# DJjjjhao/FIRA-ICSE

Measured on AMD Instinct MI355X. Metric: training commits/sec (FIRA default config), higher is better.
Workload: dtype f32; 1 GPU; BASELINE configs[1]: FIRA training step (fwd+bwd+Adam, dropout 0.1/0.2), batch 32 commits/GPU, fp32, 650-node graphs (mean nnz 1066/graph), vocab 24650; global_batch=32, parallelism=dp1

## Files before the change

### fira_icse_amd/csrc/attention.hip

```cpp
#include "engine.h"
#include "epilogue.h"
#include "mfma_frag.h"

namespace fira {

constexpr float SQRT_DH = 5.656854249492381f;
constexpr float INV_SQRT_DH = 1.0f / SQRT_DH;
constexpr int MAX_TK = 384;

constexpr float LOG2E = 1.4426950408889634f;
constexpr float SCORE2 = INV_SQRT_DH * LOG2E;
constexpr float MASKED2 = -1e9f * LOG2E;
__device__ __forceinline__ constexpr int acc_c(int s) { return (s & 3) + 8 * (s >> 2); }
__device__ __forceinline__ uint32_t low_bits(int n) { return n <= 0 ? 0u : (n >= 32 ? 0xffffffffu : (1u << n) - 1u); }
__device__ __forceinline__ float bit_select(int sel, float a, float b) {
    return __int_as_float((sel & __float_as_int(a)) | (~sel & __float_as_int(b)));
}
__device__ __forceinline__ int bit_of(uint32_t word, int c) { return __builtin_amdgcn_sbfe((int)word, c, 1); }

__device__ __forceinline__ void buf_frag(float (&f)[16], rsrc_t r, unsigned off) {
#pragma unroll
    for (int i = 0; i < 4; ++i) {
        const f32x4v v = __builtin_bit_cast(f32x4v, __builtin_amdgcn_raw_buffer_load_b128(r, off + 16u * i, 0, 0));
        f[4 * i + 0] = v.x; f[4 * i + 1] = v.y; f[4 * i + 2] = v.z; f[4 * i + 3] = v.w;
    }
}
__device__ __forceinline__ void buf_rows(float (&f)[16], rsrc_t r, unsigned off0, unsigned ld4) {
#pragma unroll
    for (int s = 0; s < 16; ++s) f[s] = buf_load_f32(r, off0 + (unsigned)acc_c(s) * ld4);
}
__device__ __forceinline__ rsrc_t rows_rsrc(const float* base, int n, int ld) {
    return buf_rsrc(base, n > 0 ? (unsigned)(n - 1) * (unsigned)ld * 4u + 128u : 0u);
}

struct AttnRanges { int qb, tq, k0, tk; };
// ... 646 lines not shown
                       ldv, key_valid, causal, q_pos0, O, ldo, kb, kvb, qpk, q_off, self_kv, k_off)
    if (Tk <= 32) { if (bf16) FIRA_ATT_FWD(1, true); else FIRA_ATT_FWD(1, false); }
    else { if (bf16) FIRA_ATT_FWD(12, true); else FIRA_ATT_FWD(12, false); }
#undef FIRA_ATT_FWD
    FIRA_CHECK_LAUNCH("attention_fwd");
    return 0;
}
int attention_fwd(hipStream_t s, int B, int H, int Tq, int Tk, const float* Q, int ldq, const float* K, int ldk,
                  const float* V, int ldv, const int32_t* key_valid, int causal, int q_pos0, float* O, int ldo,
                  const int32_t* q_off, int self_kv, int bf16, const int32_t* k_off) {
    return attention_fwd_ex(s, B, H, Tq, Tk, Q, ldq, K, ldk, V, ldv, key_valid, causal, q_pos0, O, ldo, Tk, Tk, 1, q_off, self_kv,
                            bf16, k_off);
}

int attention_bwd(hipStream_t s, int B, int H, int Tq, int Tk, const float* Q, int ldq, const float* K, int ldk,
                  const float* V, int ldv, const int32_t* key_valid, int causal, int q_pos0, const float* O, int ldo,
                  const float* dO, int lddo, float* dQ, int lddq, float* dK, int lddk, float* dV, int lddv,
                  const int32_t* q_off, int self_kv, int bf16, const int32_t* k_off) {
    ProfScope prof(s, PROF_ATTN, 0.0);
    if (B <= 0) return 0;
    if (int e = check_geometry("attention_bwd", Tq, Tk, ldq, ldk, ldv, Q, K, V)) return e;
    FIRA_REQUIRE(ldo % 4 == 0 && lddo % 4 == 0 && (uintptr_t)O % 16 == 0 && (uintptr_t)dO % 16 == 0,
                 "attention_bwd: O/dO rows must be 16-byte aligned");
#define FIRA_ATT_BWD(NW_, BF_)                                                                                      \
    hipLaunchKernelGGL((attention_bwd_kernel<NW_, BF_>), dim3(B * H), dim3(NW_ * 64), 0, s, H, Tq, Tk, Q, ldq, K, ldk, V, \
                       ldv, key_valid, causal, q_pos0, O, ldo, dO, lddo, dQ, lddq, dK, lddk, dV, lddv, q_off, self_kv, k_off)
    if (Tk <= 32) { if (bf16) FIRA_ATT_BWD(1, true); else FIRA_ATT_BWD(1, false); }
    else { if (bf16) FIRA_ATT_BWD(12, true); else FIRA_ATT_BWD(12, false); }
#undef FIRA_ATT_BWD
    FIRA_CHECK_LAUNCH("attention_bwd");
    return 0;
}

}

extern "C" {
int fira_attention_fwd(void* stream, int B, int H, int Tq, int Tk, const float* Q, int ldq, const float* K, int ldk,
                       const float* V, int ldv, const int32_t* key_valid, int causal, int q_pos0, float* O, int ldo) {
    return fira::attention_fwd((hipStream_t)stream, B, H, Tq, Tk, Q, ldq, K, ldk, V, ldv, key_valid, causal, q_pos0, O,
                               ldo);
}
int fira_decode_attention(void* stream, int BR, int H, int Tk, const float* Q, int ldq, const float* K, int ldk,
                          const float* V, int ldv, const int32_t* key_valid, float* O, int ldo, int kb, int kvb, int qpk,
                          const float* Knew, const float* Vnew, int ldn, float* Kc_out, float* Vc_out,
                          const int32_t* k_off) {
    FIRA_REQUIRE(Q && K && V && key_valid && O, "fira_decode_attention: null pointer argument");
    return fira::decode_attention((hipStream_t)stream, BR, H, Tk, Q, ldq, K, ldk, V, ldv, key_valid, O, ldo, kb, kvb, qpk, Knew,
                                  Vnew, ldn, Kc_out, Vc_out, k_off);
}
int fira_attention_bwd(void* stream, int B, int H, int Tq, int Tk, const float* Q, int ldq, const float* K, int ldk,
                       const float* V, int ldv, const int32_t* key_valid, int causal, int q_pos0, const float* O,
                       int ldo, const float* dO, int lddo, float* dQ, int lddq, float* dK, int lddk, float* dV,
                       int lddv) {
    return fira::attention_bwd((hipStream_t)stream, B, H, Tq, Tk, Q, ldq, K, ldk, V, ldv, key_valid, causal, q_pos0, O,
                               ldo, dO, lddo, dQ, lddq, dK, lddk, dV, lddv);
}
int fira_attention_fwd_ex(void* stream, int B, int H, int Tq, int Tk, const float* Q, int ldq, const float* K, int ldk,
                          const float* V, int ldv, const int32_t* key_valid, int causal, int q_pos0, float* O, int ldo,
                          const int32_t* q_off, int self_kv, int dtype, const int32_t* k_off) {
    FIRA_REQUIRE(dtype == FIRA_F32 || dtype == FIRA_BF16, "fira_attention_fwd_ex: dtype must be FIRA_F32 or FIRA_BF16");
    FIRA_REQUIRE(!(k_off && self_kv), "fira_attention_fwd_ex: k_off (ragged memory rows) and self_kv exclude each other");
    return fira::attention_fwd((hipStream_t)stream, B, H, Tq, Tk, Q, ldq, K, ldk, V, ldv, key_valid, causal, q_pos0, O,
                               ldo, q_off, self_kv, dtype == FIRA_BF16, k_off);
}
int fira_attention_bwd_ex(void* stream, int B, int H, int Tq, int Tk, const float* Q, int ldq, const float* K, int ldk,
                          const float* V, int ldv, const int32_t* key_valid, int causal, int q_pos0, const float* O,
// ... 9 lines not shown
```

### fira_icse_amd/csrc/engine.h

```cpp
#pragma once
#include "common.h"
#include <string>
#include <vector>

namespace fira {

int gemm_f32(hipStream_t s, int tA, int tB, int M, int N, int K, const float* A, int lda, const float* B, int ldb,
             float* C, int ldc, const float* bias, int flags, int splitk);
int gemm_f32_ex(hipStream_t s, int tA, int tB, int M, int N, int K, const float* A, int lda, const float* B, int ldb,
                float* C, int ldc, const float* bias, int flags, int splitk, float* colsum,
                const int32_t* c_rows = nullptr, const float* relu_mask = nullptr);
int gemm_bf16_ex(hipStream_t s, int tA, int tB, int M, int N, int K, const float* A, int lda, const float* B, int ldb,
                 float* C, int ldc, const float* bias, int flags, int splitk, float* colsum,
                 const int32_t* c_rows = nullptr, const float* relu_mask = nullptr);
struct ShadowEntry { int64_t offset; int rows, cols, pitch_t; int64_t offset_t; };
constexpr int SHADOW_MAX = 64;
struct ShadowTable {
    int n = 0;
    int64_t wbt_elems = 0;
    int tile_start[SHADOW_MAX + 1] = {0};
    ShadowEntry e[SHADOW_MAX];
};
int weight_shadows(hipStream_t s, const ShadowTable& tab, const float* P, uint16_t* Wb, uint16_t* WbT);
int gemm_bf16_wb_ex(hipStream_t s, int M, int N, int K, const float* A, int lda, const uint16_t* Bb, int ldb, float* C,
// ... 133 lines not shown
int node_features(hipStream_t s, int Nc, const int32_t* node_rows, int N, int L, int S, const int32_t* sou,
                  const int32_t* sub, const int32_t* ast, const float* emb, const float* ast_emb, const float* pos_code,
                  float* X, const int32_t* slot2 = nullptr, float* X2 = nullptr,
                  const AdamRowsView* vw = nullptr);
int rows_move(hipStream_t s, int mode, int R, int W, float* out, const float* in, const int32_t* src, const int32_t* dst);
int rows_move_ld(hipStream_t s, int mode, int R, int W, float* out, int ld_out, const float* in, int ld_in,
                 const int32_t* src, const int32_t* dst);
int rows_gather_idx(hipStream_t s, int R, float* compact, const float* src, const int32_t* rows);
int rows_scatter_add_idx(hipStream_t s, int R, const float* compact, float* dst, const int32_t* rows);
int fill_pos_tables(hipStream_t s, int L, float* pos_code, int T, float* pos_tar);
int tar_mask(hipStream_t s, int n, const int32_t* tar, int32_t* valid);
int permute_cache(hipStream_t s, int nl, int BR, int T, int len, const int32_t* parent, const float* ksrc,
                  const float* vsrc, float* kdst, float* vdst, const int32_t* hist_src, int32_t* hist_dst);
int mark_history(hipStream_t s, int BR, int T, int step, const int32_t* tokens, int32_t* hist);
int decode_embed(hipStream_t s, int BR, int T, int step, const int32_t* tokens, const float* table, const float* pos_row,
                 float* x, int32_t* hist);

int attention_fwd(hipStream_t s, int B, int H, int Tq, int Tk, const float* Q, int ldq, const float* K, int ldk,
                  const float* V, int ldv, const int32_t* key_valid, int causal, int q_pos0, float* O, int ldo,
                  const int32_t* q_off = nullptr, int self_kv = 0,
                  int bf16 = 0,
                  const int32_t* k_off = nullptr);
int attention_fwd_ex(hipStream_t s, int B, int H, int Tq, int Tk, const float* Q, int ldq, const float* K, int ldk,
                     const float* V, int ldv, const int32_t* key_valid, int causal, int q_pos0, float* O, int ldo,
                     int kb, int kvb, int qpk, const int32_t* q_off = nullptr, int self_kv = 0, int bf16 = 0,
                     const int32_t* k_off = nullptr);
int decode_attention(hipStream_t s, int BR, int H, int Tk, const float* Q, int ldq, const float* K, int ldk,
                     const float* V, int ldv, const int32_t* key_valid, float* O, int ldo, int kb, int kvb, int qpk,
                     const float* Knew = nullptr, const float* Vnew = nullptr, int ldn = 0, float* Kc_out = nullptr,
                     float* Vc_out = nullptr, const int32_t* k_off = nullptr);
int decode_self_block(hipStream_t s, int BR, int Tk, int T, const float* qkv, float* Kc, float* Vc, const int32_t* hist,
                      const float* WoT, const float* bo, const float* xres, const float* gamma, const float* beta,
                      const float* WqT, const float* bq, float* xa, float* qc);
int decode_attention_kv16(hipStream_t s, int BR, int H, int Tk, const float* Q, int ldq, const uint16_t* K, int ldk,
                          const uint16_t* V, int ldv, const int32_t* key_valid, float* O, int ldo, int kb, int kvb, int qpk,
                          const int32_t* k_off = nullptr);
int rows_to_bf16(hipStream_t s, int64_t n, const float* in, uint16_t* out);
int rows_from_bf16(hipStream_t s, int64_t n, const uint16_t* in, float* out);
int attention_bwd(hipStream_t s, int B, int H, int Tq, int Tk, const float* Q, int ldq, const float* K, int ldk,
                  const float* V, int ldv, const int32_t* key_valid, int causal, int q_pos0, const float* O, int ldo,
                  const float* dO, int lddo, float* dQ, int lddq, float* dK, int lddk, float* dV, int lddv,
                  const int32_t* q_off = nullptr, int self_kv = 0, int bf16 = 0, const int32_t* k_off = nullptr);
int copy_score_fwd(hipStream_t s, int B, int T, int S, const float* src, const float* tgt, const float* w,
                   const float* bias, float* score);
int copy_score_fwd_ex(hipStream_t s, int B, int T, int S, const float* src, const float* tgt, const float* w,
                      const float* bias, float* score, int qpk, const int32_t* mem_valid,
                      const int32_t* tar_label = nullptr, int V = 0,
                      const int32_t* t_off = nullptr);
int copy_score_bwd_ex(hipStream_t s, int B, int T, int S, const float* src, const float* tgt, const float* w,
                      const float* dscore, float* dsrc, float* dtgt, float* dw, float* dbias, const int32_t* mem_valid,
                      float* part = nullptr, const int32_t* t_off = nullptr);
int copy_score_bwd_blocks(int B, int S);
constexpr int COPY_PART_STRIDE = 264;
int decode_dist(hipStream_t s, int R, int V, int S, const float* logits, int ldl, const float* score,
                const int32_t* mem_valid, int qpk, const float* gate_logits, float* dist, int32_t* best_id,
                float* best_p, const float* x = nullptr, const float* wp = nullptr, const float* bp = nullptr);
int inv_count(hipStream_t s, const int32_t* n_tok, float* out);
int sample_dist(hipStream_t s, int R, int n_sample, int V, int S, const float* logits, int ldl, const float* score,
                const int32_t* mem_valid, const float* x, const float* wp, const float* bp, int T, int step,
                const int32_t* key, const uint64_t* seed_dev, float temperature, int top_k, float top_p, float* dist,
                int32_t* best_id, float* best_p);
int score_dist(hipStream_t s, int R, int n_cand, int V, int L, int S, const float* logits, int ldl, const float* score,
               const int32_t* mem_valid, const float* x, const float* wp, const float* bp, const int32_t* target,
               const int32_t* label, const int32_t* sou, const int32_t* sub, float* dist, float* p_word, float* p_entry,
               int32_t* entry, float* copy_share, float* p_label, int32_t* top_id, float* logp_word, float* logp_entry,
               float* logp_label);
// ... 69 lines not shown
```

### fira_icse_amd/csrc/engine.hip

```cpp
#include "engine.h"
#include <hip/hip_ext.h>
#include "epilogue.h"
#include <stdlib.h>
#include <map>
#include <mutex>

namespace fira {

static int64_t shadow_wbt_elems(const Layout& L);

struct Arena {
    char* base;
    size_t used = 0;
    explicit Arena(void* b) : base((char*)b) {}
    template <typename T>
    T* get(size_t n) {
        size_t bytes = (n * sizeof(T) + 255) / 256 * 256;
        T* p = base ? (T*)(base + used) : nullptr;
        used += bytes;
        return p;
    }
    float* f(size_t n) { return get<float>(n); }
};

// ... 5 lines not shown
};

struct EncGrad {
    float *dY2, *dYc, *dqk;
};
struct DecGrad {
    float *dYf, *dh, *dYc, *dq, *dYs, *dqkv;
};


static constexpr int KV_ROW_PAD = 64;

struct Plan {
    int B, NB, CB, MB, TB, N, L, S, A, T, V, ldl, nl, F;
    int kvp;
    float *pos_code, *pos_tar;
    int32_t *mem_valid, *tar_valid, *compact_row, *iota, *code_slot, *mem_slot, *row_bt, *rows_c;
    int32_t *mem_off, *mem_valid_c;
    std::vector<float*> X;
    std::vector<EncSave> enc;
    std::vector<DecSave> dec;
    std::vector<EncGrad> encg;
    std::vector<DecGrad> decg;
    float *vtab_all, *H, *mem, *mem_c, *src_c, *x0, *kv_all, *src, *tgt, *score, *gate, *dec_c, *logits;
    float *W21, *c21, *rsum;
    float *W21t;
    uint16_t *W21x = nullptr, *W21tx = nullptr;
    uint16_t *WcX = nullptr, *WcTX = nullptr;
    uint16_t* WkvX = nullptr;
    float* WkvT = nullptr;
    uint16_t* WkvTX = nullptr;
    uint16_t* WoutTX = nullptr;
    uint16_t *xh_planes = nullptr;
    float *WcT;
    float *dW21, *dc21;
    float *inv_ntok;
    float *dXa, *dXb, *dNB2, *dCB_a, *dvtab_all;
    float *zero_beg = nullptr, *zero_end = nullptr;
    uint16_t *wb = nullptr, *wbt = nullptr;
    uint16_t *w21b = nullptr, *w21bt = nullptr;
    float* red_buf = nullptr;
    size_t red_cap = 0;
    float* panel_scratch = nullptr;
    size_t panel_floats = 0;
    float *dmem_c, *dsrc, *dsrc_c, *dtgt, *dkv_all, *ddec, *ddec_c, *dT_a, *dT_c;

    size_t build(void* ws, const fira_dims& d, int B_, bool training) {
        Arena a(ws);
        B = B_; L = d.sou_len; S = d.sub_len; A = d.ast_len; T = d.tar_len; V = d.vocab; nl = d.n_layer; F = d.d_ff;
        N = L + S + A;
        NB = B * N; CB = B * L; MB = B * (L + S); TB = B * T;
        ldl = (V + 63) / 64 * 64;
        const size_t D = FIRA_D;
        pos_code = a.f((size_t)L * D);
        pos_tar = a.f((size_t)T * D);
        mem_valid = a.get<int32_t>((size_t)MB);
        tar_valid = a.get<int32_t>((size_t)TB);
        compact_row = a.get<int32_t>((size_t)TB);
        iota = a.get<int32_t>((size_t)TB);
        row_bt = a.get<int32_t>((size_t)TB);
        rows_c = a.get<int32_t>((size_t)TB);
        code_slot = a.get<int32_t>((size_t)NB);
        mem_slot = a.get<int32_t>((size_t)NB);
        mem_off = a.get<int32_t>((size_t)B + 1);
        mem_valid_c = a.get<int32_t>((size_t)MB);
        inv_ntok = a.f(64);
        {
            const Layout* lay = get_layout(&d);
            const size_t tot = lay ? (size_t)lay->total : 0;
            wb = a.get<uint16_t>(tot);
            wbt = a.get<uint16_t>((lay ? (size_t)shadow_wbt_elems(*lay) : 0) + 64);
            w21b = a.get<uint16_t>((size_t)nl * D * D);
            w21bt = a.get<uint16_t>((size_t)nl * D * D + 64);
        }
        X.resize(nl + 1);
        for (int l = 0; l <= nl; ++l) X[l] = a.f((size_t)NB * D);
        enc.resize(nl);
        for (int l = 0; l < nl; ++l) {
            EncSave& e = enc[l];
            e.Xc = a.f((size_t)CB * D); e.qk = a.f((size_t)CB * 2 * D); e.c = a.f((size_t)CB * D);
            e.s1 = a.f((size_t)CB * D); e.st1 = a.f((size_t)CB * 2);
            e.Z = a.f((size_t)NB * D); e.s2 = a.f((size_t)NB * D); e.st2 = a.f((size_t)NB * 2);
        }
        vtab_all = a.f((size_t)4 * nl * D);
        W21 = a.f((size_t)nl * D * D); c21 = a.f((size_t)nl * D); rsum = a.f((size_t)NB);
        W21t = a.f((size_t)nl * D * D);
        W21x = a.get<uint16_t>((size_t)nl * 3 * D * D);
        W21tx = a.get<uint16_t>((size_t)nl * 3 * D * D);
        WcX = a.get<uint16_t>((size_t)nl * 9 * D * D);
        WcTX = a.get<uint16_t>((size_t)nl * 9 * D * D);
        WkvX = a.get<uint16_t>((size_t)nl * 6 * D * D);
        WkvT = a.f((size_t)nl * 2 * D * D);
        WkvTX = a.get<uint16_t>((size_t)nl * 6 * D * D);
        WoutTX = a.get<uint16_t>((size_t)cdiv(V, D) * 3 * D * D);
        xh_planes = a.get<uint16_t>(head_logits_x3_scratch_elems(TB));
        WcT = a.f((size_t)nl * 3 * D * D);
        H = a.f((size_t)NB * D);
        mem = a.f((size_t)MB * D);
        mem_c = a.f((size_t)MB * D);
        src_c = a.f((size_t)MB * D);
        x0 = a.f((size_t)TB * D);
        kvp = nl * 2 * D + KV_ROW_PAD;
        kv_all = a.f((size_t)MB * kvp);
        dec.resize(nl);
        for (int l = 0; l < nl; ++l) {
            DecSave& e = dec[l];
            e.qkv = a.f((size_t)TB * 3 * D); e.ao = a.f((size_t)TB * D); e.s_a = a.f((size_t)TB * D);
            e.st_a = a.f((size_t)TB * 2); e.x_a = a.f((size_t)TB * D); e.qc = a.f((size_t)TB * D);
            e.ao2 = a.f((size_t)TB * D); e.s_c = a.f((size_t)TB * D); e.st_c = a.f((size_t)TB * 2);
            e.x_c = a.f((size_t)TB * D); e.h = a.f((size_t)TB * F); e.s_f = a.f((size_t)TB * D);
            e.st_f = a.f((size_t)TB * 2); e.x_f = a.f((size_t)TB * D);
        }
        src = a.f((size_t)MB * D); tgt = a.f((size_t)TB * D);
        score = a.f((size_t)TB * (L + S)); gate = a.f((size_t)TB * 2);
        dec_c = a.f((size_t)TB * D); logits = a.f((size_t)TB * ldl);
        if (training) {
            dXa = a.f((size_t)NB * D); dXb = a.f((size_t)NB * D); dNB2 = a.f((size_t)NB * D);
            dCB_a = a.f((size_t)CB * D);
            red_cap = (size_t)nl * ((size_t)cdiv(NB, 16) * 4 * D + (size_t)cdiv(CB, 16) * 2 * D)
                    + (size_t)3 * nl * cdiv(TB, 16) * 2 * D
                    + (size_t)nl * std::max((size_t)cdiv(CB, 16) * 4 * D, (size_t)comb_fused_bwd_parts() * 6 * D + 64)
                    + (size_t)cdiv(L + S, 16) * B * COPY_PART_STRIDE + 4096;
            red_buf = a.f(red_cap);
            panel_floats = (size_t)320 * 256 * 256;
            panel_scratch = a.f(panel_floats);
            zero_beg = (float*)a.get<char>(0);
            dvtab_all = a.f((size_t)4 * nl * D);
            dW21 = a.f((size_t)nl * D * D + (size_t)nl * D); dc21 = dW21 + (size_t)nl * D * D;
// ... 438 lines not shown
    const float* P;
    float* G;
    Plan* pl;
    float p_drop, p_gcn;
    uint64_t seed;
    int R = 0;
    const int32_t* rows = nullptr;
    int Td = 0;
    const int32_t* dec_off = nullptr;
    const int32_t* row_bt = nullptr;
    const int32_t* rows_dense = nullptr;
    bool deferred = false;
    bool kv_ragged = false;
    bool serial = false;
    float* loss_sum = nullptr;
    int32_t* n_tok = nullptr;
    hipEvent_t ev_kv[16] = {};
    int kv_waited = 0;
    hipEvent_t ev_src = nullptr;
    hipEvent_t ev_zero = nullptr;
    const fira_adam_opts* adam = nullptr;
    float* Pw = nullptr;
    bool dp_begin = false;
    bool wout_planes = false;
    bool kv_planes = false;
    int32_t* row_step = nullptr;
    fira_adam_opts rows_ad{};
    bool adam_a_only = false;
    hipEvent_t ev_early = nullptr;
    const float* count = nullptr;
    const ClipStep* clip = nullptr;
    const ShadowTable* shadow_tab = nullptr;
    hipEvent_t ev_shadow = nullptr;
    int n_lanes = 1;
    struct Lane { hipStream_t s; int b0, nb, r0, nr; } lanes[2] = {};
};
typedef Ctx::Lane Lane;

static AdamRowsTables adam_rows_tables(const Layout& L, float* params, const fira_adam_opts& ad, int32_t* row_step) {
    AdamRowsTables tb;
    tb.p = params; tb.m = ad.m; tb.v = ad.v;
    tb.off[0] = L.dec_emb; tb.off[1] = L.emb;
    tb.rows[0] = tb.rows[1] = L.d.vocab;
    tb.last = row_step;
    return tb;
}

static int decoder_lanes(Ctx& c) {
    constexpr int DEC_LANES_MIN_ROWS = 768;
    static const int forced = [] { const char* e = getenv("FIRA_DEC_LANES"); return e ? (atoi(e) >= 2 ? 2 : 1) : 0; }();
    const int want = forced ? forced : (c.Td >= DEC_LANES_MIN_ROWS ? 2 : 1);
    c.n_lanes = g_lanes = 1;
    c.lanes[0] = Lane{c.s, 0, c.pl->B, 0, c.Td};
    const fira_batch& bt = *c.bt;
    if (want < 2 || !c.dec_off || !bt.dec_off_host || bt.B < 2 || !side_on() || c.serial || !c.kv_ragged) return 0;
    SideStream& sd = side();
    if (!sd.lane) {
        if (hipStreamCreateWithFlags(&sd.lane, hipStreamNonBlocking) != hipSuccess) return set_err("lane stream: create failed");
    }
    int bm = 1, best = 1 << 30;
    for (int b = 1; b < bt.B; ++b) {
        const int d = abs(2 * bt.dec_off_host[b] - c.Td);
        if (d < best) { best = d; bm = b; }
    }
    const int rm = bt.dec_off_host[bm];
    if (rm <= 0 || rm >= c.Td || bt.dec_off_host[bt.B] != c.Td) return 0;
    c.n_lanes = g_lanes = 2;
    c.lanes[0] = Lane{c.s, 0, bm, 0, rm};
    c.lanes[1] = Lane{sd.lane, bm, bt.B - bm, rm, c.Td - rm};
    return 0;
}
static int lanes_fork(Ctx& c) {
    for (int k = 1; k < c.n_lanes; ++k) {
        hipEvent_t e = side().ev();
        if (hipEventRecord(e, c.s) != hipSuccess || hipStreamWaitEvent(c.lanes[k].s, e, 0) != hipSuccess) return set_err("lane fork failed");
    }
    return 0;
}
static int lanes_join(Ctx& c) {
    for (int k = 1; k < c.n_lanes; ++k) {
        hipEvent_t e = side().ev();
        if (hipEventRecord(e, c.lanes[k].s) != hipSuccess || hipStreamWaitEvent(c.s, e, 0) != hipSuccess) return set_err("lane join failed");
    }
    return 0;
}
static int lanes_fork_to(Ctx& c, hipStream_t target) {
    for (int k = 0; k < c.n_lanes; ++k) {
        hipEvent_t e = side().ev();
        if (hipEventRecord(e, c.lanes[k].s) != hipSuccess || hipStreamWaitEvent(target, e, 0) != hipSuccess) return set_err("lane -> side stream fork failed");
    }
    return 0;
}

static inline bool fold_one_launch(int nl) { return nl <= 10; }
static inline bool comb_x3_on(int nl) { return nl <= 8; }
static inline bool gcn_x3_on(int nl) { return gcn_fused_on() && fold_one_launch(nl); }
static inline bool kv_x3_on(int nl) { return nl * 2 <= 24; }

static int adam_rows_prefetch(Ctx& c, hipStream_t st) {
    const fira_batch& bt = *c.bt;
    const Plan& p = *c.pl;
    const fira_adam_opts& ad = c.rows_ad;
    AdamRowsLists ls{};
    auto add = [&](const int32_t* ids, int n, int table) {
        if (!ids || n <= 0) return;
        const int k = ls.n_lists++;
        ls.ids[k] = ids; ls.table[k] = table;
        ls.end[k] = (k ? ls.end[k - 1] : 0) + n;
    };
    add(bt.tar, p.B * p.T, 0);
    return adam_rows_catchup(st, adam_rows_tables(*c.L, const_cast<float*>(c.P), ad, c.row_step), &ls, ad.lr, ad.beta1, ad.beta2, ad.eps,
                             ad.step - 1);
}

static int encoder_forward(Ctx& c, bool defer_memory_proj) {
    Plan& p = *c.pl;
    const Layout& L = *c.L;
    const fira_batch& bt = *c.bt;
    hipStream_t s = c.s;
    const int D = FIRA_D, Nc = bt.n_nodes, Cc = bt.n_code, Mc = bt.n_mem, KV = p.nl * 2 * D;
    hipEvent_t ev_fold0 = nullptr, ev_fold = nullptr, ev_comb = nullptr;
    bool fold_waited = false;
    {
// ... 34 lines not shown
                uint16_t* dst[24];
                int n = 0;
                for (int l = 0; l < p.nl; ++l) {
                    src[n] = p.W21 + (size_t)l * D * D; dst[n++] = p.W21x + (size_t)l * 3 * D * D;
                    if (c.G) { src[n] = p.W21t + (size_t)l * D * D; dst[n++] = p.W21tx + (size_t)l * 3 * D * D; }
                }
                TRY(gcn_split_planes(fs, n, src, dst));
            }
            if (ax && (!g_Wb || gcn_fused_on())) TRY(side_mark(&ev_fold0));
        } else
        for (int l = 0; l < p.nl; ++l) {
            const EncLayer& w = L.enc[l];
            TRY(gemm_f32_ex(fs, 0, 0, D, D, D, c.P + w.fc2w, D, c.P + w.fc1w, D, p.W21 + (size_t)l * D * D, D, nullptr, 0, 0, nullptr));
            TRY(gemm_f32_ex(fs, 0, 1, D, 1, D, c.P + w.fc2w, D, c.P + w.fc1b, D, p.c21 + (size_t)l * D, 1, nullptr, 0, 0, nullptr));
            if (l == 0 && gcn_fused_on()) TRY(transpose256(fs, 1, p.W21, p.W21t));
            if (ax && l == 0 && !g_Wb && p.nl > 1) TRY(side_mark(&ev_fold0));
        }
        if (g_Wb) {
            ShadowTable t21;
            for (int l = 0; l < p.nl && l < SHADOW_MAX; ++l) {
                t21.e[l] = ShadowEntry{(int64_t)l * D * D, D, D, D, (int64_t)l * D * D};
                t21.tile_start[l + 1] = t21.tile_start[l] + cdiv(D, 64) * cdiv(D, 64);
                t21.n = l + 1;
            }
            TRY(weight_shadows(fs, t21, p.W21, p.w21b, p.w21bt));
            g_W21 = p.W21; g_W21n = (int64_t)p.nl * D * D; g_W21b = p.w21b; g_W21bT = p.w21bt;
        }
        if (!fold_one && gcn_fused_on() && p.nl > 1) TRY(transpose256(fs, p.nl - 1, p.W21 + (size_t)D * D, p.W21t + (size_t)D * D));
        if (ax && !(ev_fold0 && fold_one && gcn_fused_on())) TRY(side_mark(&ev_fold));
        if (!ev_fold0) ev_fold0 = ev_fold;
        if (c.shadow_tab) {
            TRY(weight_shadows(fs, *c.shadow_tab, c.P, p.wb, p.wbt));
            if (ax) TRY(side_mark(&c.ev_shadow));
        }
    }
    const int32_t* head_list = c.dec_off ? c.rows_dense : c.rows;
    TRY(prep(s, p.B, p.L, p.S, p.T, bt.sou, bt.sub_token, bt.tar, p.mem_valid, bt.tar ? p.tar_valid : nullptr, p.pos_code,
             p.pos_tar, c.R, head_list, bt.tar ? p.compact_row : nullptr, head_list ? nullptr : p.iota, c.loss_sum, c.n_tok,
             Nc, bt.code_rows, Cc, p.code_slot, bt.mem_rows, Mc, p.mem_slot, c.dec_off, p.row_bt, p.rows_c, bt.mem_dst,
             p.mem_off, p.mem_valid_c));
    c.kv_ragged = true;
    AdamRowsView vw_emb;
    if (c.row_step)
        vw_emb = adam_rows_view(adam_rows_tables(L, nullptr, c.rows_ad, c.row_step), 1, c.rows_ad.lr, c.rows_ad.beta1, c.rows_ad.beta2,
                                c.rows_ad.eps, c.rows_ad.step - 1);
    TRY(node_features(s, Nc, bt.node_rows, p.N, p.L, p.S, bt.sou, bt.sub_token, bt.ast_change, c.P + L.emb, c.P + L.ast_emb,
                      p.pos_code, p.X[0], p.code_slot, p.enc[0].Xc, &vw_emb));
    TRY(linear(s, 4, p.nl * D, D, c.P + L.mark_emb, D, c.P + L.w2_all, c.P + L.b2_all, p.vtab_all, p.nl * D));
    for (int l = 0; l < p.nl; ++l) {
        const EncLayer& w = L.enc[l];
        EncSave& e = p.enc[l];
        float* X = p.X[l];
        if (l < 8) {
            if (l == 0 && ev_comb) TRY(main_wait(s, ev_comb, __LINE__));
            else if (l == 0 && ev_fold0) { TRY(main_wait(s, ev_fold0, __LINE__)); fold_waited = true; }
            const float* wt = p.WcT + (size_t)l * 3 * D * D;
            TRY(comb_fused_fwd(s, Cc, e.Xc, wt, wt + (size_t)D * D, wt + (size_t)2 * D * D, c.P + w.bqk, c.P + w.bo,
                               p.vtab_all + l * D, p.nl * D, bt.code_mark, e.qk, e.c, c.P + w.ln1g, c.P + w.ln1b, e.s1, X,
                               bt.code_rows, e.st1, c.p_drop, c.seed, site(l, SITE_GATE), site(l, SITE_COMB_OUT), g_dtype == 1,
                               comb_x3_on(p.nl) ? p.WcX + (size_t)l * 9 * D * D : nullptr));
        } else {
        TRY(linear(s, Cc, 2 * D, D, e.Xc, D, c.P + w.wqk, c.P + w.bqk, e.qk, 2 * D));
        TRY(combination_fwd(s, Cc, e.qk, p.vtab_all + l * D, p.nl * D, bt.code_mark, e.c, c.p_drop, c.seed, site(l, SITE_GATE)));
        TRY(linear_ln(s, Cc, D, e.c, D, c.P + w.wo, c.P + w.bo, e.Xc, c.P + w.ln1g, c.P + w.ln1b, e.s1, X, e.st1, c.p_drop,
                      c.seed, site(l, SITE_COMB_OUT), bt.code_rows));
        }
// ... 56 lines not shown
        }
        c.deferred = true;
        return 0;
    }
    TRY(gemm_any(s, 0, 1, Mc, KV, D, p.mem_c, D, c.P + L.wkv_all, D, p.kv_all, p.kvp, c.P + L.bkv_all, 0, 0, nullptr));
    TRY(gemm_any(s, 0, 1, Mc, D, D, p.mem_c, D, c.P + L.ws, D, p.src, D, nullptr, 0, 0, nullptr, bt.mem_dst));
    return 0;
}

static int decoder_forward(Ctx& c) {
    Plan& p = *c.pl;
    const Layout& L = *c.L;
    const int D = FIRA_D, H = L.d.n_head, Sm = p.L + p.S;
    if (c.row_bt) {
        AdamRowsView vw;
        if (c.row_step)
            vw = adam_rows_view(adam_rows_tables(L, nullptr, c.rows_ad, c.row_step), 0, c.rows_ad.lr, c.rows_ad.beta1, c.rows_ad.beta2,
                                c.rows_ad.eps, c.rows_ad.step - 1);
        TRY(embed_rows_fwd(c.s, c.Td, p.T, c.row_bt, c.bt->tar, c.P + L.dec_emb, p.pos_tar, p.x0, &vw));
    } else {
        if (c.row_step) TRY(adam_rows_prefetch(c, c.s));
        TRY(embed_gather_fwd(c.s, p.B, p.T, c.bt->tar, c.P + L.dec_emb, p.pos_tar, p.x0, p.T, 0));
    }
    ProfDecoderTag prof_tag;
    TRY(decoder_lanes(c));
    ProfScope prof_region(c.s, PROF_DEC_REGION, 0.0);
    TRY(lanes_fork(c));
    struct LaneState {
        const float *x = nullptr, *pend_sum = nullptr, *pend_g = nullptr, *pend_b = nullptr;
        float *pend_y = nullptr, *pend_st = nullptr;
        int kv_waited = 0;
    } state[2];
    for (int k = 0; k < c.n_lanes; ++k) state[k].x = p.x0;
    for (int l = 0; l < p.nl; ++l) {
        const DecLayer& w = L.dec[l];
        DecSave& e = p.dec[l];
        const bool last = l + 1 == p.nl;
        for (int k = 0; k < c.n_lanes; ++k) {
            const Lane& ln = c.lanes[k];
            LaneState& st = state[k];
            hipStream_t s = ln.s;
            const size_t r0 = (size_t)ln.r0;
            const int nr = ln.nr;
            const uint32_t idx0 = (uint32_t)(r0 * D);
            auto consume = [&](int N, const float* W, const float* b, float* Y, int flags) -> int {
                if (st.pend_sum) {
                    int rc = 0;
                    float* sum = const_cast<float*>(st.pend_sum) + r0 * D;
                    const bool fused = gemm_tile32_ln_try(s, nr, N, sum, D, W, b, Y + r0 * N, N, flags, st.pend_g, st.pend_b,
                                                          st.pend_y + r0 * D, st.pend_st + r0 * 2, &rc);
                    if (!fused)
                        rc = add_layernorm_fwd(s, nr, sum, nullptr, st.pend_g, st.pend_b, st.pend_y + r0 * D, st.pend_st + r0 * 2, 0.f, 0, 0,
                                               nullptr);
                    st.pend_sum = nullptr;
                    if (rc || fused) return rc;
                }
                return linear(s, nr, N, D, st.x + r0 * D, D, W, b, Y + r0 * N, N, flags);
            };
            auto close_block = [&](int K, const float* X, const float* W, const float* b, const float* res, const float* g,
                                   const float* be, float* sum, float* y, float* stt, uint32_t site_id, bool may_defer,
                                   const int32_t* slot2, float* y2, int n2, const int32_t* rows2) -> int {
                int rc = 0;
                if (may_defer && linear_presum(s, nr, K, X + r0 * K, K, W, b, res + r0 * D, sum + r0 * D, c.p_drop, c.seed, site_id,
                                               &rc, idx0)) {
                    st.pend_sum = sum; st.pend_g = g; st.pend_b = be; st.pend_y = y; st.pend_st = stt;
                    return rc;
                }
                return linear_ln(s, nr, K, X + r0 * K, K, W, b, res + r0 * D, g, be, sum + r0 * D, y + r0 * D, stt + r0 * 2, c.p_drop,
                                 c.seed, site_id, nullptr, nullptr, nullptr, slot2 ? slot2 + r0 : nullptr, y2, n2, rows2, idx0);
            };
            const int32_t* q_off = c.dec_off ? c.dec_off + ln.b0 : nullptr;
            TRY(consume(3 * D, c.P + w.wqkv, c.P + w.bqkv, e.qkv, 0));
            TRY(attention_fwd(s, ln.nb, H, p.T, p.T, e.qkv, 3 * D, e.qkv + D, 3 * D, e.qkv + 2 * D, 3 * D, p.tar_valid + (size_t)ln.b0 * p.T,
                              1, 0, e.ao, D, q_off, 1, attn_bf16()));
            TRY(close_block(D, e.ao, c.P + w.wo_s, c.P + w.bo_s, st.x, c.P + w.lns_g, c.P + w.lns_b, e.s_a, e.x_a, e.st_a,
                            site(l, SITE_SELF), true, nullptr, nullptr, 0, nullptr));
            st.x = e.x_a;
            TRY(consume(D, c.P + w.wq_c, c.P + w.bq_c, e.qc, 0));
            if (c.deferred) {
                int m = l;
                while (m < p.nl - 1 && c.ev_kv[m] == nullptr) ++m;
                if (c.ev_kv[m] != nullptr && st.kv_waited < m + 1) {
                    TRY(main_wait(s, c.ev_kv[m], __LINE__));
                    st.kv_waited = m + 1;
                }
            }
            TRY(attention_fwd(s, ln.nb, H, p.T, Sm, e.qc, D, p.kv_all + l * 2 * D, p.kvp, p.kv_all + l * 2 * D + D, p.kvp,
                              c.kv_ragged ? p.mem_valid_c : p.mem_valid, 0, 0, e.ao2, D, q_off, 0, attn_bf16(),
                              c.kv_ragged ? p.mem_off + ln.b0 : nullptr));
            TRY(close_block(D, e.ao2, c.P + w.wo_c, c.P + w.bo_c, e.x_a, c.P + w.lnc_g, c.P + w.lnc_b, e.s_c, e.x_c, e.st_c,
                            site(l, SITE_CROSS), true, nullptr, nullptr, 0, nullptr));
            st.x = e.x_c;
            TRY(consume(p.F, c.P + w.w1, c.P + w.b1, e.h, FIRA_GEMM_RELU));
            const bool head_copy = last && c.rows != nullptr && c.R > 0;
            TRY(close_block(p.F, e.h, c.P + w.w2, c.P + w.b2, e.x_c, c.P + w.lnf_g, c.P + w.lnf_b, e.s_f, e.x_f, e.st_f,
                            site(l, SITE_FFN), !last, head_copy ? p.compact_row : nullptr, head_copy ? p.dec_c : nullptr,
                            head_copy ? c.R : 0, head_copy ? c.rows : nullptr));
            st.x = e.x_f;
        }
    }
    TRY(lanes_join(c));
    return 0;
}

static int head_forward(Ctx& c, int R, const int32_t* rows, float* loss_sum, int32_t* n_tok, int32_t* argmax_out,
                        int want_grad) {
    Plan& p = *c.pl;
    const Layout& L = *c.L;
    hipStream_t s = c.s;
// ... 1030 lines not shown
```

Baseline: 13740 commits/s.

## Fuse decoder self-attention block into one per-sequence kernel

Adds a kernel that, per target sequence, applies the pending LayerNorm, runs the QKV projection, causal self-attention over all 8 heads, and the output projection with dropout and residual. Weights come from pre-split x3 bf16 planes that are prepared once per step on the side stream. This replaces the separate QKV GEMM, attention and output-projection launches with one, cutting launch count and intermediate round trips through global memory for short decoder sequences (T<=32). In exchange it adds per-step weight-plane conversion work and an event dependency, and runs only with one lane and in fp32 mode.

New measurement: 13280 commits/s. 0.966x the previous value.

```diff
diff --git a/fira_icse_amd/csrc/attention.hip b/fira_icse_amd/csrc/attention.hip
--- a/fira_icse_amd/csrc/attention.hip
+++ b/fira_icse_amd/csrc/attention.hip
@@ -1,6 +1,7 @@
 #include "engine.h"
 #include "epilogue.h"
 #include "mfma_frag.h"
+#include "x3.h"
 
 namespace fira {
 
@@ -713,6 +714,262 @@
     return 0;
 }
 
+constexpr int DB_WAVES = 8;
+constexpr int DB_ROWS = 32;
+constexpr size_t DB_PLANE = (size_t)DB_ROWS * 512;
+typedef float db_acc __attribute__((ext_vector_type(4)));
+struct DecSelfArgs {
+    int T, Td;
+    const float* x;
+    const float *ln_sum, *ln_g, *ln_b;
+    float *ln_y, *ln_st;
+    const uint16_t* Wx;
+    const float *bqkv, *bo;
+    float *qkv, *ao, *s_out;
+    const int32_t* q_off;
+    const int32_t* key_valid;
+    float p, inv_keep;
+    uint64_t seed;
+    uint32_t site;
+};
+__device__ __forceinline__ void db_units(uint4 (&b)[2][3], rsrc_t rW, unsigned xl, int ks) {
+#pragma unroll
+    for (int u = 0; u < 2; ++u)
+#pragma unroll
+        for (int pl = 0; pl < 3; ++pl)
+            b[u][pl] = __builtin_bit_cast(uint4, __builtin_amdgcn_raw_buffer_load_b128(rW, xl + (unsigned)u * 8192u,
+                                                                                       pl * (int)GX_WPLANE + ks * 1024, 0));
+}
+__device__ __forceinline__ void db_product(const char* __restrict__ sm_p, int a_q, const uint16_t* __restrict__ Wx, unsigned xl, int nt,
+                                           uint4 (&bx)[2][3], db_acc (&acc)[2][2], const uint16_t* __restrict__ Wnext) {
+    const rsrc_t rW = buf_rsrc(Wx, 3u * (unsigned)GX_WPLANE);
+    const rsrc_t rN = buf_rsrc(Wnext ? Wnext : Wx, 3u * (unsigned)GX_WPLANE);
+    uint4 b[2][2][3];
+#pragma unroll
+    for (int u = 0; u < 2; ++u)
+#pragma unroll
+        for (int pl = 0; pl < 3; ++pl) b[0][u][pl] = bx[u][pl];
+#pragma unroll
+    for (int ks = 0; ks < 8; ++ks) {
+        if (ks + 1 < 8) db_units(b[(ks + 1) & 1], rW, xl, ks + 1);
+        else if (Wnext) db_units(b[0], rN, xl, 0);
+        asm volatile("" ::: "memory");
+#pragma unroll
+        for (int tt = 0; tt < 2; ++tt) {
+            if (tt < nt) {
+#pragma unroll
+                for (int u = 0; u < 2; ++u)
+                    gx_terms<3>(acc[u][tt], sm_p + ((a_q ^ (ks << 6)) + tt * 8192), DB_PLANE, b[ks & 1][u]);
+            }
+        }
+        asm volatile("" ::: "memory");
+    }
+#pragma unroll
+    for (int u = 0; u < 2; ++u)
+#pragma unroll
+        for (int pl = 0; pl < 3; ++pl) bx[u][pl] = b[0][u][pl];
+}
+
+__global__ __launch_bounds__(DB_WAVES * 64) void decoder_self_block_kernel(const DecSelfArgs a) {
+    __shared__ __attribute__((aligned(16))) char sm_p[3 * DB_PLANE];
+    const int b = blockIdx.x, t = threadIdx.x, lane = t & 63, wave = t >> 6;
+    const int l15 = lane & 15, kq = lane >> 4, l31 = lane & 31, kh = lane >> 5;
+    const AttnRanges rg = attn_ranges(a.q_off, nullptr, b, b, a.T, a.T, true, lane);
+    const int qb = rg.qb, tq = min(rg.tq, DB_ROWS);
+    if (tq <= 0) return;
+    const int nt = tq > 16 ? 2 : 1;
+    constexpr int D = FIRA_D;
+    constexpr size_t WX = 3 * (size_t)D * D;
+    const unsigned xl = gx_wlane(2 * wave, lane);
+    const int a_q = gx_frag_base(l15, kq);
+    uint4 bx[2][3];
+    db_units(bx, buf_rsrc(a.Wx, 3u * (unsigned)GX_WPLANE), xl, 0);
+    asm volatile("" ::: "memory");
+    {
+        constexpr int RPW = DB_ROWS / DB_WAVES;
+        const float* src = a.ln_sum ? a.ln_sum : a.x;
+        f32x4v x[RPW], g, be;
+#pragma unroll
+        for (int i = 0; i < RPW; ++i)
+            x[i] = *reinterpret_cast<const f32x4v*>(src + (size_t)(qb + min(wave * RPW + i, tq - 1)) * D + lane * 4);
+        if (a.ln_sum) {
+            g = *reinterpret_cast<const f32x4v*>(a.ln_g + lane * 4);
+            be = *reinterpret_cast<const f32x4v*>(a.ln_b + lane * 4);
+#pragma unroll
+            for (int i = 0; i < RPW; ++i) {
+                const int row = wave * RPW + i;
+                const float mean = wave_sum((x[i].x + x[i].y) + (x[i].z + x[i].w)) * (1.0f / D);
+                const f32x4v d = x[i] - mean;
+                const float var = wave_sum((d.x * d.x + d.y * d.y) + (d.z * d.z + d.w * d.w)) * (1.0f / D);
+                const float rstd = 1.0f / sqrtf(var + 1e-5f);
+                x[i] = (x[i] - mean) * rstd * g + be;
+                if (row < tq) {
+                    *reinterpret_cast<f32x4v*>(a.ln_y + (size_t)(qb + row) * D + lane * 4) = x[i];
+                    if (lane == 0) { a.ln_st[2 * (size_t)(qb + row)] = mean; a.ln_st[2 * (size_t)(qb + row) + 1] = rstd; }
+                }
+            }
+        }
+#pragma unroll
+        for (int i = 0; i < RPW; ++i) {
+            const int row = wave * RPW + i;
+            gx_store_row4<3>(sm_p, DB_PLANE, row, lane, row < tq ? x[i] : f32x4v{0.f, 0.f, 0.f, 0.f});
+        }
+    }
+    lds_barrier();
+    {
+        const rsrc_t rO = buf_rsrc(a.qkv, (unsigned)((size_t)a.Td * 3 * D * 4));
+        for (int blk = 0; blk < 3; ++blk) {
+            db_acc acc[2][2];
+#pragma unroll
+            for (int u = 0; u < 2; ++u)
+#pragma unroll
+                for (int tt = 0; tt < 2; ++tt) acc[u][tt] = db_acc{0.f, 0.f, 0.f, 0.f};
+            float bias[2];
+#pragma unroll
+            for (int u = 0; u < 2; ++u) bias[u] = a.bqkv[blk * D + (2 * wave + u) * 16 + l15];
+            db_product(sm_p, a_q, a.Wx + blk * WX, xl, nt, bx, acc, a.Wx + (blk + 1) * WX);
+#pragma unroll
+            for (int tt = 0; tt < 2; ++tt) {
+                if (tt < nt) {
+#pragma unroll
+                    for (int u = 0; u < 2; ++u)
+#pragma unroll
+                        for (int r = 0; r < 4; ++r) {
+                            const int row = tt * 16 + 4 * kq + r, col = blk * D + (2 * wave + u) * 16 + l15;
+                            const unsigned o = row < tq ? ((unsigned)(qb + row) * (unsigned)(3 * D) + (unsigned)col) * 4u : FIRA_OOB;
+                            __builtin_amdgcn_raw_buffer_store_b32(__builtin_bit_cast(unsigned, acc[u][tt][r] + bias[u]), rO, o, 0, 0);
+                        }
+                }
+            }
+        }
+    }
+    __syncthreads();
+    {
+        const int h = wave;
+        const int ld = 3 * D;
+        const rsrc_t rQ = rows_rsrc(a.qkv + (size_t)qb * ld + h * FIRA_DH, tq, ld);
+        const rsrc_t rK = rows_rsrc(a.qkv + (size_t)qb * ld + D + h * FIRA_DH, tq, ld);
+        const rsrc_t rV = rows_rsrc(a.qkv + (size_t)qb * ld + 2 * D + h * FIRA_DH, tq, ld);
+        const rsrc_t rA = rows_rsrc(a.ao + (size_t)qb * D + h * FIRA_DH, tq, D);
+        const rsrc_t rM = buf_rsrc(a.key_valid + (size_t)b * a.T, (unsigned)tq * 4u);
+        float bq[16], ak[16], vv[16];
+        buf_frag(bq, rQ, (unsigned)l31 * (unsigned)ld * 4u + (unsigned)kh * 64u);
+        buf_frag(ak, rK, (unsigned)l31 * (unsigned)ld * 4u + (unsigned)kh * 64u);
+        buf_rows(vv, rV, (unsigned)(4 * kh) * (unsigned)ld * 4u + (unsigned)l31 * 4u, (unsigned)ld * 4u);
+        const int kvld = __builtin_amdgcn_raw_buffer_load_b32(rM, (unsigned)l31 * 4u, 0, 0);
+        const TileMask tm = tile_mask(kvld, tq, kh);
+        const uint32_t maskedT = ~tm.valid | ~low_bits(l31 - 4 * kh + 1);
+        f32x16 st;
+        float mx = -INFINITY;
+        if (tm.live) {
+#pragma unroll
+            for (int s = 0; s < 16; ++s) vv[s] = bit_select(bit_of(tm.valid, acc_c(s)), vv[s], 0.f);
+            f32x16 acc;
+#pragma unroll
+            for (int r = 0; r < 16; ++r) acc[r] = 0.f;
+            acc = chain16<false>(ak, bq, acc);
+#pragma unroll
+            for (int r = 0; r < 16; ++r) {
+                float x = bit_select(bit_of(maskedT, acc_c(r)), MASKED2, acc[r] * SCORE2);
+                x = bit_select(bit_of(tm.outside, acc_c(r)), -INFINITY, x);
+                st[r] = x;
+                mx = fmaxf(mx, x);
+            }
+        } else {
+#pragma unroll
+            for (int r = 0; r < 16; ++r) {
+                const float x = bit_select(bit_of(tm.outside, acc_c(r)), -INFINITY, MASKED2);
+                st[r] = x;
+                mx = fmaxf(mx, x);
+            }
+        }
+        mx = fmaxf(mx, __shfl_xor(mx, 32, 64));
+        float sum = 0.f;
+#pragma unroll
+        for (int r = 0; r < 16; ++r) {
+            const float pr = __builtin_amdgcn_exp2f(st[r] - mx);
+            st[r] = pr;
+            sum += pr;
+        }
+        sum += __shfl_xor(sum, 32, 64);
+        const float inv_sum = 1.0f / sum;
+        f32x16 o;
+#pragma unroll
+        for (int r = 0; r < 16; ++r) o[r] = 0.f;
+        if (tm.live) {
+            float pn[16];
+#pragma unroll
+            for (int s = 0; s < 16; ++s) pn[s] = st[s] * inv_sum;
+            o = chain16<false>(pn, vv, o);
+        }
+#pragma unroll
+        for (int r = 0; r < 16; ++r) {
+            const int row = 4 * kh + acc_c(r);
+            __builtin_amdgcn_raw_buffer_store_b32(__float_as_int(o[r]), rA, (unsigned)row * (unsigned)D * 4u + (unsigned)l31 * 4u, 0, 0);
+            if (row < nt * 16) gx_store_elem<3>(sm_p, DB_PLANE, row, h * FIRA_DH + l31, row < tq ? o[r] : 0.f);
+        }
+    }
+    {
+        const float* res = a.ln_sum ? a.ln_y : a.x;
+        const rsrc_t rR = buf_rsrc(res, (unsigned)((size_t)a.Td * D * 4));
+        const rsrc_t rS = buf_rsrc(a.s_out, (unsigned)((size_t)a.Td * D * 4));
+        float bias[2], rv[2][2][4];
+        unsigned off[2][2][4];
+#pragma unroll
+        for (int u = 0; u < 2; ++u) {
+            const int col = (2 * wave + u) * 16 + l15;
+            bias[u] = a.bo[col];
+#pragma unroll
+            for (int tt = 0; tt < 2; ++tt)
+#pragma unroll
+                for (int r = 0; r < 4; ++r) {
+                    const int row = tt * 16 + 4 * kq + r;
+                    off[u][tt][r] = row < tq ? ((unsigned)(qb + row) * (unsigned)D + (unsigned)col) * 4u : FIRA_OOB;
+                    rv[u][tt][r] = buf_load_f32(rR, off[u][tt][r]);
+                }
+        }
+        __syncthreads();
+        db_acc acc[2][2];
+#pragma unroll
+        for (int u = 0; u < 2; ++u)
+#pragma unroll
+            for (int tt = 0; tt < 2; ++tt) acc[u][tt] = db_acc{0.f, 0.f, 0.f, 0.f};
+        db_product(sm_p, a_q, a.Wx + 3 * WX, xl, nt, bx, acc, nullptr);
+#pragma unroll
+        for (int tt = 0; tt < 2; ++tt) {
+            if (tt < nt) {
+#pragma unroll
+                for (int u = 0; u < 2; ++u)
+#pragma unroll
+                    for (int r = 0; r < 4; ++r) {
+                        const int row = tt * 16 + 4 * kq + r, col = (2 * wave + u) * 16 + l15;
+                        float v = acc[u][tt][r] + bias[u];
+                        if (a.p > 0.f) v *= dropout_scale(a.seed, a.site, (uint32_t)(qb + row) * D + (uint32_t)col, a.p, a.inv_keep);
+                        v += rv[u][tt][r];
+                        __builtin_amdgcn_raw_buffer_store_b32(__builtin_bit_cast(unsigned, v), rS, off[u][tt][r], 0, 0);
+                    }
+            }
+        }
+    }
+}
+
+int decoder_self_block(hipStream_t s, int B, int T, int Td, const float* x, const float* ln_sum, const float* ln_g, const float* ln_b,
+                       float* ln_y, float* ln_st, const uint16_t* Wx, const float* bqkv, const float* bo, float* qkv, float* ao,
+                       float* s_out, const int32_t* q_off, const int32_t* key_valid, float p_drop, uint64_t seed, uint32_t site) {
+    FIRA_REQUIRE((x || ln_sum) && Wx && bqkv && bo && qkv && ao && s_out && key_valid, "decoder_self_block: null pointer argument");
+    FIRA_REQUIRE(!ln_sum || (ln_g && ln_b && ln_y && ln_st), "decoder_self_block: LayerNorm arguments missing");
+    FIRA_REQUIRE(T >= 1 && T <= DB_ROWS && Td >= 1 && (size_t)Td * 3 * FIRA_D * 4 < (1ull << 31), "decoder_self_block: bad geometry");
+    if (B <= 0) return 0;
+    ProfScope prof(s, PROF_GEMM, 2.0 * Td * 4.0 * FIRA_D * FIRA_D, 4.0 * ((double)Td * FIRA_D * 7 + 4.0 * FIRA_D * FIRA_D));
+    DecSelfArgs a;
+    a.T = T; a.Td = Td; a.x = x; a.ln_sum = ln_sum; a.ln_g = ln_g; a.ln_b = ln_b; a.ln_y = ln_y; a.ln_st = ln_st;
+    a.Wx = Wx; a.bqkv = bqkv; a.bo = bo; a.qkv = qkv; a.ao = ao; a.s_out = s_out; a.q_off = q_off; a.key_valid = key_valid;
+    a.p = p_drop; a.inv_keep = p_drop > 0.f ? 1.0f / (1.0f - p_drop) : 1.0f; a.seed = seed; a.site = site;
+    hipLaunchKernelGGL(decoder_self_block_kernel, dim3(B), dim3(DB_WAVES * 64), 0, s, a);
+    FIRA_CHECK_LAUNCH("decoder_self_block");
+    return 0;
+}
+
 }
 
 extern "C" {
diff --git a/fira_icse_amd/csrc/engine.h b/fira_icse_amd/csrc/engine.h
--- a/fira_icse_amd/csrc/engine.h
+++ b/fira_icse_amd/csrc/engine.h
@@ -189,6 +189,9 @@
 int decode_self_block(hipStream_t s, int BR, int Tk, int T, const float* qkv, float* Kc, float* Vc, const int32_t* hist,
                       const float* WoT, const float* bo, const float* xres, const float* gamma, const float* beta,
                       const float* WqT, const float* bq, float* xa, float* qc);
+int decoder_self_block(hipStream_t s, int B, int T, int Td, const float* x, const float* ln_sum, const float* ln_g, const float* ln_b,
+                       float* ln_y, float* ln_st, const uint16_t* Wx, const float* bqkv, const float* bo, float* qkv, float* ao,
+                       float* s_out, const int32_t* q_off, const int32_t* key_valid, float p_drop, uint64_t seed, uint32_t site);
 int decode_attention_kv16(hipStream_t s, int BR, int H, int Tk, const float* Q, int ldq, const uint16_t* K, int ldk,
                           const uint16_t* V, int ldv, const int32_t* key_valid, float* O, int ldo, int kb, int kvb, int qpk,
                           const int32_t* k_off = nullptr);
diff --git a/fira_icse_amd/csrc/engine.hip b/fira_icse_amd/csrc/engine.hip
--- a/fira_icse_amd/csrc/engine.hip
+++ b/fira_icse_amd/csrc/engine.hip
@@ -61,6 +61,7 @@
     uint16_t* WkvTX = nullptr;
     uint16_t* WoutTX = nullptr;
     uint16_t *xh_planes = nullptr;
+    uint16_t* WdX = nullptr;
     float *WcT;
     float *dW21, *dc21;
     float *inv_ntok;
@@ -123,6 +124,7 @@
         WkvTX = a.get<uint16_t>((size_t)nl * 6 * D * D);
         WoutTX = a.get<uint16_t>((size_t)cdiv(V, D) * 3 * D * D);
         xh_planes = a.get<uint16_t>(head_logits_x3_scratch_elems(TB));
+        WdX = a.get<uint16_t>((size_t)nl * 12 * D * D);
         WcT = a.f((size_t)nl * 3 * D * D);
         H = a.f((size_t)NB * D);
         mem = a.f((size_t)MB * D);
@@ -627,6 +629,8 @@
     const ClipStep* clip = nullptr;
     const ShadowTable* shadow_tab = nullptr;
     hipEvent_t ev_shadow = nullptr;
+    bool dec_planes = false;
+    hipEvent_t ev_decx = nullptr;
     int n_lanes = 1;
     struct Lane { hipStream_t s; int b0, nb, r0, nr; } lanes[2] = {};
 };
@@ -684,6 +688,30 @@
         hipEvent_t e = side().ev();
         if (hipEventRecord(e, c.lanes[k].s) != hipSuccess || hipStreamWaitEvent(target, e, 0) != hipSuccess) return set_err("lane -> side stream fork failed");
     }
+    return 0;
+}
+
+static bool dec_blocks_fit(const Ctx& c) {
+    static const bool off = [] { const char* e = getenv("FIRA_DEC_BLOCKS"); return e && e[0] == '0'; }();
+    const fira_dims& d = c.L->d;
+    return !off && g_dtype == 0 && d.d_model == FIRA_D && d.n_head == 8 && c.pl->T <= 32 && c.pl->nl <= 12 &&
+           (size_t)c.pl->TB * 3 * FIRA_D * 4 < (1ull << 31);
+}
+static int dec_block_planes(Ctx& c, hipStream_t st) {
+    const Plan& p = *c.pl;
+    const size_t DD = (size_t)FIRA_D * FIRA_D;
+    const float* src[48];
+    uint16_t* dst[48];
+    int n = 0;
+    for (int l = 0; l < p.nl; ++l) {
+        const DecLayer& w = c.L->dec[l];
+        for (int j = 0; j < 4; ++j) {
+            src[n] = j < 3 ? c.P + w.wqkv + j * DD : c.P + w.wo_s;
+            dst[n++] = p.WdX + ((size_t)l * 4 + j) * 3 * DD;
+        }
+    }
+    TRY(gcn_split_planes(st, n, src, dst));
+    c.dec_planes = true;
     return 0;
 }
 
@@ -784,6 +812,10 @@
         if (c.shadow_tab) {
             TRY(weight_shadows(fs, *c.shadow_tab, c.P, p.wb, p.wbt));
             if (ax) TRY(side_mark(&c.ev_shadow));
+        }
+        if (dec_blocks_fit(c)) {
+            TRY(dec_block_planes(c, fs));
+            if (ax) TRY(side_mark(&c.ev_decx));
         }
     }
     const int32_t* head_list = c.dec_off ? c.rows_dense : c.rows;
@@ -906,6 +938,11 @@
         int kv_waited = 0;
     } state[2];
     for (int k = 0; k < c.n_lanes; ++k) state[k].x = p.x0;
+    const bool blocks = c.n_lanes == 1 && H * FIRA_DH == D && dec_blocks_fit(c);
+    if (blocks) {
+        if (!c.dec_planes) TRY(dec_block_planes(c, c.s));
+        else if (c.ev_decx) TRY(main_wait(c.s, c.ev_decx, __LINE__));
+    }
     for (int l = 0; l < p.nl; ++l) {
         const DecLayer& w = L.dec[l];
         DecSave& e = p.dec[l];
@@ -944,11 +981,18 @@
                                  c.seed, site_id, nullptr, nullptr, nullptr, slot2 ? slot2 + r0 : nullptr, y2, n2, rows2, idx0);
             };
             const int32_t* q_off = c.dec_off ? c.dec_off + ln.b0 : nullptr;
+            if (blocks) {
+                TRY(decoder_self_block(s, ln.nb, p.T, c.Td, st.x, st.pend_sum, st.pend_g, st.pend_b, st.pend_y, st.pend_st,
+                                       p.WdX + (size_t)l * 12 * D * D, c.P + w.bqkv, c.P + w.bo_s, e.qkv, e.ao, e.s_a, q_off,
+                                       p.tar_valid, c.p_drop, c.seed, site(l, SITE_SELF)));
+                st.pend_sum = e.s_a; st.pend_g = c.P + w.lns_g; st.pend_b = c.P + w.lns_b; st.pend_y = e.x_a; st.pend_st = e.st_a;
+            } else {
             TRY(consume(3 * D, c.P + w.wqkv, c.P + w.bqkv, e.qkv, 0));
             TRY(attention_fwd(s, ln.nb, H, p.T, p.T, e.qkv, 3 * D, e.qkv + D, 3 * D, e.qkv + 2 * D, 3 * D, p.tar_valid + (size_t)ln.b0 * p.T,
                               1, 0, e.ao, D, q_off, 1, attn_bf16()));
             TRY(close_block(D, e.ao, c.P + w.wo_s, c.P + w.bo_s, st.x, c.P + w.lns_g, c.P + w.lns_b, e.s_a, e.x_a, e.st_a,
                             site(l, SITE_SELF), true, nullptr, nullptr, 0, nullptr));
+            }
             st.x = e.x_a;
             TRY(consume(D, c.P + w.wq_c, c.P + w.bq_c, e.qc, 0));
             if (c.deferred) {
```
